# Boey-li/AdaptiGraph

Measured on AMD Instinct MI355X. Metric: rollout graph-steps/s (batch x rollout steps / wall; edge build + GNN forward + state update per graph-step), higher is better.
Workload: dtype f16+fp8corr+bf16x3; 1 GPU; rope 1000+tool particles, batch 256/GPU, 10-step rollout (BASELINE configs[1]); global_batch=256, rollout_steps=10, parallelism=batch-shard x1 + all-gather, rollout_streams=1, weights=seed-0 random init (reference default init), precision=fast, model_status=0, self_edges=1, agg_q16=1

## Files before the change

adaptigraph_amd/csrc/ag_api.hip:

```cpp
#include "../../include/adaptigraph_hip.h"
#include "ag_common.h"

#include <cmath>
#include <cstdarg>
#include <cstdio>
#include <cstdlib>
#include <cstring>
#include <string>
#include <utility>
#include <vector>

namespace {

thread_local std::string g_err;

int fail(int code, const char *fmt, ...)
{
    char buf[512];
    va_list ap;
    va_start(ap, fmt);
    vsnprintf(buf, sizeof buf, fmt, ap);
    va_end(ap);
    g_err = buf;
    return code;
// ... 172 lines not shown
                }
            }
        }
    }
}

}

#define AG_MAX_PARTS 4
struct ag_model {
    ag_model_config cfg;
    float *dev = nullptr;
    size_t dev_floats = 0;
    AgWeights w{};
    int split = 0, fuse_agg = 0, precision = 2, max_blocks = 512, edge_products = 2, edge_ws = 1, node_ws = 1, agg_q16 = 1, node_dedup = 1, self_edges = 1,
        shared_state = 0;
    bool h2_ok = true;
    hipStream_t aux_stream[4] = {nullptr, nullptr, nullptr, nullptr};
    hipEvent_t ev_fork = nullptr, ev_join[4] = {nullptr, nullptr, nullptr, nullptr};
    int cu_split = 0;
    int n_cus = 256;
    int part_cus = 0;
    hipStream_t mfma_stream = nullptr, hbm_stream = nullptr;
    hipEvent_t ev_ready[4] = {nullptr, nullptr, nullptr, nullptr}, ev_enc[4] = {nullptr, nullptr, nullptr, nullptr}, ev_join_mfma = nullptr;
    bool profiling = false;
    std::vector<std::pair<hipEvent_t, hipEvent_t>> ev[AG_K_COUNT];
    size_t ev_used[AG_K_COUNT] = {0, 0, 0, 0, 0, 0};
    unsigned long long *edge_counter = nullptr;
    int *status = nullptr;
};

// ... 222 lines not shown
        r.hs_q16 = (path.q16 && p > 0) ? 1 : 0;
        r.hs_out_q16 = v.hs_q16;
        r.agg_q16 = v.agg_q16;
        if (path.agg_launch) { Timed t(m, AG_K_AGGREGATE, s); ag_launch_aggregate(r, path, last, s); }
        { Timed t(m, AG_K_NODE_UPDATE, s); ag_launch_node_update(m->w, r, path, last, s); }
        std::swap(a.hr, a.hr_out);
        std::swap(a.hs, a.hs_out);
    }
}

struct Option {
    const char *name, *env;
    int ag_model::*field;
    int (*accept)(const ag_model *m, int v);
    const char *takes;
};
int flag(const ag_model *, int v) { return v != 0; }
const Option kOptions[] = {
    {"rollout_streams", "AG_SPLIT", &ag_model::split, [](const ag_model *, int v) { return v >= 0 && v <= AG_MAX_PARTS ? v : -1; }, "0 (by the workload) or 1..4"},
    {"fuse_aggregate", "AG_FUSE_AGG", &ag_model::fuse_agg, [](const ag_model *, int v) { return v == 0 || v == 2 ? v : -1; }, "0 (separate launch) or 2 (reduce inside node_update)"},
    {"precision", "AG_PRECISION", &ag_model::precision, [](const ag_model *, int v) { return v >= 0 && v <= 2 ? v : -1; }, "0 (f32), 1 (bf16x3) or 2 (fast)"},
    {"max_blocks", "AG_MAX_BLOCKS", &ag_model::max_blocks, [](const ag_model *, int v) { return v >= 1 ? v : -1; }, "a positive workgroup count"},
    {"edge_products", "AG_EDGE_PRODUCTS", &ag_model::edge_products, [](const ag_model *, int v) { return v == 2 || v == 3 ? v : -1; }, "2 (fp16 edge stack) or 3 (split-bf16)"},
    {"edge_stationary", "AG_EDGE_WS", &ag_model::edge_ws, flag, "any integer (0 = off)"},
    {"node_stationary", "AG_NODE_WS", &ag_model::node_ws, flag, "any integer (0 = off)"},
    {"agg_q16", "AG_AGG_Q16", &ag_model::agg_q16, flag, "any integer (0 = off)"},
    {"node_dedup", "AG_NODE_DEDUP", &ag_model::node_dedup, [](const ag_model *, int v) { return v < 0 ? 0 : (v > 2 ? 2 : v); }, "any integer (clamped to 0..2)"},
    {"self_edges", "AG_SELF_EDGES", &ag_model::self_edges, flag, "any integer (0 = off)"},
    {"shared_state", "AG_SHARED_STATE", &ag_model::shared_state, flag, "any integer (0 = off)"},
    {"cu_split", "AG_CU_SPLIT", &ag_model::cu_split, [](const ag_model *m, int v) { return v == 0 || (v >= 8 && v <= m->n_cus - 8 && !(v & 7)) ? v : -1; },
     "0 (off) or a multiple of 8 in [8, #CUs - 8]"},
};

const Option *find_option(const char *name)
{
    for (const Option &o : kOptions)
        if (!strcmp(name, o.name)) return &o;
    return nullptr;
}

int load_env_options(ag_model *m)
{
    static const char *const kPrecisionNames[] = {"f32", "bf16x3", "fast"};
    for (const Option &o : kOptions) {
        const char *text = getenv(o.env);
        if (!text) continue;
        char *end = nullptr;
        long long v = strtoll(text, &end, 10);
        bool parsed = *text && !*end && v == (int)v;
        for (int i = 0; i < 3 && !parsed && o.field == &ag_model::precision; ++i)
            if (!strcmp(text, kPrecisionNames[i])) { v = i; parsed = true; }
        const int stored = parsed ? o.accept(m, (int)v) : -1;
        if (stored < 0) return fail(AG_ERR_CONFIG, "%s=%s: %s takes %s", o.env, text, o.name, o.takes);
        m->*o.field = stored;
    }
    return AG_OK;
}

}

// ... 423 lines not shown
                   ag_stream_t stream)
{
    if (!pos || !mask || !tool_mask || !thr_sq || !row_ptr || !edge_recv || !edge_send || !workspace)
        return fail(AG_ERR_ARG, "ag_build_edges: null argument");
    if (B < 1 || N < 1 || topk < 1 || topk > 64) return fail(AG_ERR_ARG, "ag_build_edges: B=%d N=%d topk=%d (1..64)", B, N, topk);
    if (variant != AG_VARIANT_SINGLE && variant != AG_VARIANT_BATCH) return fail(AG_ERR_ARG, "bad variant %d", variant);
    if ((int64_t)B * N >= (1ll << 31) / 64) return fail(AG_ERR_ARG, "B*N too large for int32 edge offsets");
    if (e_cap < ag_edge_capacity(B, N, topk, connect_tools_all, max_tools))
        return fail(AG_ERR_ARG, "ag_build_edges: e_cap %lld < ag_edge_capacity()", (long long)e_cap);
    AgEdgeArgs a{};
    a.pos = pos; a.mask = mask; a.tool = tool_mask; a.thr_sq = thr_sq;
    a.topk = topk; a.connect = connect_tools_all ? 1 : 0; a.variant = variant; a.B = B; a.N = N; a.max_tools = max_tools;
    edge_caps(N, topk, a.connect, max_tools, &a.cap0, &a.cap);
    a.row_ptr = row_ptr; a.edge_recv = edge_recv; a.edge_send = edge_send;
    a.pos_stride = (size_t)N * 3;
    Carver c(workspace, workspace_bytes);
    carve_edges(c, a);
    if (!c.ok()) return fail(AG_ERR_WS, "ag_build_edges: workspace %zu < %zu bytes", workspace_bytes, c.off);
    ag_launch_build_edges(a, static_cast<hipStream_t>(stream));
    AG_HIP(hipGetLastError());
    return AG_OK;
}

size_t ag_forward_workspace_bytes(int B, int N, int64_t e_cap) { return ag_forward_workspace_bytes_for(nullptr, B, N, e_cap); }

size_t ag_forward_workspace_bytes_for(const ag_model *m, int B, int N, int64_t e_cap)
{
    AgFwdArgs a{};
    Carver c(nullptr, 0);
    carve_forward(c, a, B, N, e_cap, resolve_path(m, B, N, 0).q16);
// ... 289 lines not shown
        AG_HIP(hipStreamWaitEvent(sE, m->ev_fork, 0));
        AG_HIP(hipStreamWaitEvent(sR, m->ev_fork, 0));
    }
    int rc = AG_OK;
    struct Run { AgStepArgs st{}; hipStream_t s; } run[AG_MAX_PARTS];
    for (int k = 0; k < parts && rc == AG_OK; ++k) {
        Part &q = part[k];
        hipStream_t s = partitioned ? sR : (k == 0 ? s0 : m->aux_stream[k]);
        run[k].s = s;
        const size_t b0 = (size_t)q.b0;
        const size_t state_bytes = (size_t)q.B * H * plane * sizeof(float);
        if (hipMemcpyAsync(q.state, state0 + b0 * H * plane, state_bytes, hipMemcpyDeviceToDevice, s) != hipSuccess) { rc = AG_ERR_HIP; break; }
        AgEdgeArgs &e = q.e;
        AgFwdArgs &f = q.f;
        e.mask = mask + b0 * N; e.tool = tool_mask + b0 * N; e.thr_sq = thr_sq + b0; e.topk = p->topk;
        e.variant = AG_VARIANT_BATCH; e.max_tools = p->max_tools;
        e.pos = q.state + (size_t)(H - 1) * plane;
        e.pos_stride = (size_t)H * plane;
        f.state = q.state; f.attrs = attrs + b0 * N * 2; f.action = delta + b0 * plane;
        f.p_instance = p_instance + b0 * n_p * p->n_instance; f.phys = phys ? phys + b0 * Pd : nullptr;
        f.row_ptr = e.row_ptr; f.edge_recv = e.edge_recv; f.edge_send = e.edge_send;
        f.pred_pos = q.pp; f.pred_motion = q.pm;
        f.B = q.B; f.N = N; f.n_p = n_p; f.n_inst = p->n_instance; f.phys_dim = Pd;
        f.pstep = m->cfg.pstep; f.clamp = m->cfg.motion_clamp;
        if (m->self_edges) {
            e.self_attrs = f.attrs; e.self_class_row0 = f.self_class_row0;
            f.self_info = e.self_info; f.self_rows = AG_SELF_ROWS;
        }
        AgStepArgs &st = run[k].st;
        st.state = q.state; st.delta = delta + b0 * plane; st.pred_pos = q.pp;
        st.obj_mask = obj_mask ? obj_mask + b0 * n_p : nullptr; st.repeat = repeat + b0;
// ... 9 lines not shown
        for (int k = 0; k < parts && rc == AG_OK && p->n_steps > 0; ++k) {
            AgFwdArgs &f = part[k].f;
            { Timed tm(m, AG_K_EDGES, sR); ag_launch_build_edges(part[k].e, sR); }
            setup_args(m, f, part[k].path, AG_MLP_WG_PER_CU * (m->n_cus - m->cu_split));
            f.ws_blocks = m->cu_split;
            run_node_encode(m, f, sR);
            run_node_encode_fallback(m, f, sR);
            rc = encode(k);
        }
        for (int ai = 1; ai <= p->n_steps && rc == AG_OK; ++ai)
            for (int k = 0; k < parts && rc == AG_OK; ++k) {
                AgFwdArgs &f = part[k].f;
                if (hipStreamWaitEvent(sR, m->ev_enc[k], 0) != hipSuccess) { rc = AG_ERR_HIP; break; }
                run_propagate(m, f, part[k].path, sR);
                run[k].st.step = ai;
                { Timed tm(m, AG_K_ROLLOUT_STEP, sR); ag_launch_rollout_step(run[k].st, sR); }
                if (ai < p->n_steps) {
                    { Timed tm(m, AG_K_EDGES, sR); ag_launch_build_edges(part[k].e, sR); }
                    if (!f.dedup) run_node_encode(m, f, sR);
                    run_node_encode_fallback(m, f, sR);
                    rc = encode(k);
                }
            }
    } else
    for (int ai = 1; ai <= p->n_steps && rc == AG_OK; ++ai)
        for (int k = 0; k < parts && rc == AG_OK; ++k) {
            hipStream_t s = run[k].s;
            AgFwdArgs &f = part[k].f;
            AgEdgeArgs &e = part[k].e;
            const AgPath &path = part[k].path;
            if (ai == 1) {
                setup_args(m, f, path, part_blocks);
                if (path.edge == AG_EDGE_H3_WS) {
                    e.tab_state = f.state; e.tab_attrs = f.attrs; e.tab_pinst = f.p_instance; e.tab_out = f.edge_node_tab;
                    e.tab_n_inst = f.n_inst; e.tab_n_p = f.n_p; e.tab_status = f.status;
                }
                if (f.dedup) { e.map_node_row = f.node_row; e.map_ovf = f.ovf; e.map_send_c = f.send_c; }
            }
            if (ai == 1 || !f.dedup) run_node_encode(m, f, s);
            int riders;
            { Timed tm(m, AG_K_EDGES, s); riders = ag_launch_build_edges(e, s); }
            f.tab_done = (riders & AG_RIDER_TAB) != 0;
            f.remap_done = (riders & AG_RIDER_MAP) != 0;
            run_node_encode_fallback(m, f, s);
            run_edge_encode(m, f, path, s);
            if (ai == 1 && k == 0 && parts > 1) {
                if (hipEventRecord(m->ev_fork, s0) != hipSuccess) { rc = AG_ERR_HIP; break; }
                for (int kk = 1; kk < parts; ++kk)
                    if (hipStreamWaitEvent(m->aux_stream[kk], m->ev_fork, 0) != hipSuccess) rc = AG_ERR_HIP;
                if (rc != AG_OK) break;
            }
            run_propagate(m, f, path, s);
            run[k].st.step = ai;
            { Timed tm(m, AG_K_ROLLOUT_STEP, s); ag_launch_rollout_step(run[k].st, s); }
        }
    for (int k = 0; k < parts && rc == AG_OK && state_final; ++k) {
        const size_t b0 = (size_t)part[k].b0;
        if (hipMemcpyAsync(state_final + b0 * H * plane, part[k].state, (size_t)part[k].B * H * plane * sizeof(float),
                           hipMemcpyDeviceToDevice, run[k].s) != hipSuccess)
            rc = AG_ERR_HIP;
    }
    if (partitioned) {
        if (hipEventRecord(m->ev_join_mfma, sE) != hipSuccess || hipStreamWaitEvent(s0, m->ev_join_mfma, 0) != hipSuccess ||
            hipEventRecord(m->ev_join[1], sR) != hipSuccess || hipStreamWaitEvent(s0, m->ev_join[1], 0) != hipSuccess)
            rc = AG_ERR_HIP;
    } else
    for (int k = 1; k < parts; ++k)
        if (hipEventRecord(m->ev_join[k], m->aux_stream[k]) != hipSuccess || hipStreamWaitEvent(s0, m->ev_join[k], 0) != hipSuccess)
            rc = AG_ERR_HIP;
// ... 7 lines not shown
```

adaptigraph_amd/csrc/ag_common.h:

```cpp
#pragma once
#include <hip/hip_runtime.h>
#include <stdint.h>

#define AG_F 150
#define AG_FP 160
#define AG_NT 5
#define AG_WSTRIDE 160
#define AG_CHUNK_FLOATS 5120
#define AG_CHUNK_F4 1280
#define AG_ROWS_PER_WAVE 32
#ifndef AG_MLP_THREADS
#define AG_MLP_THREADS 256
#endif
#define AG_MLP_WAVES (AG_MLP_THREADS / 64)
#define AG_ROWS_PER_BLOCK (32 * AG_MLP_WAVES)
#define AG_MLP_WG_PER_CU (512 / AG_MLP_THREADS)
#define AG_PACK_BLOCK (32 * AG_FP)
#define AG_NHIS 4
#define AG_ATTR 2
#define AG_EDGE_IN 17
#define AG_NODE_IN_MAX 8

enum { AG_PREC_F32 = 0, AG_PREC_B3 = 1 };
enum { AG_OK = 0, AG_ERR_ARG = -1, AG_ERR_HIP = -2, AG_ERR_WS = -3, AG_ERR_CONFIG = -4 };
// ... 264 lines not shown
    void *grid_raw;
    int32_t *cell_start;
    float4 *sorted;
    const float *tab_state, *tab_attrs, *tab_pinst;
    float *tab_out;
    int tab_n_inst, tab_n_p;
    int *tab_status;
    const int32_t *map_node_row;
    const int *map_ovf;
    int32_t *map_send_c;
    const float *self_attrs;
    int32_t *self_info;
    int32_t *self_pos;
    int self_class_row0;
    const int32_t *active;
};
enum { AG_RIDER_TAB = 1, AG_RIDER_MAP = 2 };
int ag_launch_build_edges(const AgEdgeArgs &a, hipStream_t s);

__device__ __forceinline__ void ag_edge_node_tab_row(const float *state, const float *attrs, const float *p_instance, int n_inst, int n_p,
                                                     int B, int N, float *tab, int *status, int g, long long class_row0 = -1)
{
    if (class_row0 >= 0 && g < AG_SELF_CLASSES) {
        float4 *dst = reinterpret_cast<float4 *>(tab + (size_t)(class_row0 + g) * 16);
        dst[0] = make_float4(g == 0 ? 1.0f : 0.0f, g == 0 ? 0.0f : 1.0f, 0.0f, 0.0f);
        dst[1] = dst[2] = dst[3] = make_float4(0.0f, 0.0f, 0.0f, 0.0f);
    }
    if (g >= B * N) return;
    const int b = g / N, i = g - b * N;
    float p[AG_NHIS][3];
#pragma unroll
    for (int hh = 0; hh < AG_NHIS; ++hh)
#pragma unroll
// ... 19 lines not shown

struct AgStepArgs {
    float *state;
    const float *delta;
    const float *pred_pos;
    const int32_t *cmap;
    uint8_t *dirty;
    int32_t *sample_dirty;
    const uint8_t *obj_mask;
    const int32_t *repeat;
    float *out_seq;
    int B, N, n_p, H, step, height_mode;
    float raise;
};
void ag_launch_rollout_step(const AgStepArgs &a, hipStream_t s);
void ag_launch_zero_words(int32_t *p, int n, hipStream_t s);

struct AgSharedArgs {
    int B1, N, n_p, n_inst, phys_dim, H;
    const float *state0, *delta, *attrs, *p_instance, *phys, *thr_sq;
    const uint8_t *mask, *tool, *obj_mask;
    const int32_t *repeat;
    float *s_state, *s_delta, *s_attrs, *s_pinst, *s_phys, *s_thr;
    uint8_t *s_mask, *s_tool, *s_obj_mask;
    int32_t *s_repeat;
    uint8_t *dirty;
    uint8_t *sel_a, *sel_b;
    int32_t *sample_dirty;
    int32_t *active;
    int max_tools;
// ... 47 lines not shown
```

adaptigraph_amd/csrc/ag_edges.hip:

```cpp
#include "ag_common.h"

namespace {

constexpr int kRowsPerBlock = 16;
constexpr int kCand = 384;

__device__ __forceinline__ void wave_lds_fence()
{
    asm volatile("s_waitcnt lgkmcnt(0)" ::: "memory");
    __builtin_amdgcn_wave_barrier();
}

__device__ int prune_topk(float *cd, int *cj, int cnt, int k, int lane)
{
    unsigned keepbits = 0;
    for (int base = 0, ch = 0; base < cnt; base += 64, ++ch) {
        const int idx = base + lane;
        const bool have = idx < cnt;
        const float d = have ? cd[idx] : 0.f;
        const int jj = have ? cj[idx] : 0;
        int rank = 0;
        for (int t = 0; t < cnt; ++t) {
            const float dt = cd[t];
            const int jt = cj[t];
// ... 106 lines not shown
    *total = wsum[0] + wsum[1] + wsum[2] + wsum[3];
    __syncthreads();
    return base + x - v;
}

constexpr int kCellMax = 8192;

struct GridParams { float x0, y0, z0, inv; int nx, ny, nz, total; };

__device__ __forceinline__ int cell_coord(float x, float x0, float inv, int n)
{
    const int c = (int)((x - x0) * inv);
    return c < 0 ? 0 : (c >= n ? n - 1 : c);
}

__global__ __launch_bounds__(256) void bin_kernel(AgEdgeArgs a)
{
    __shared__ int cnt[kCellMax];
    __shared__ float red[6][4];
    __shared__ GridParams G;
    if ((int)blockIdx.x >= a.B) {
        const int gt = ((int)blockIdx.x - a.B) * 256 + (int)threadIdx.x;
        if (a.active && gt < a.B * a.N && !a.active[gt / a.N]) return;
        ag_edge_node_tab_row(a.tab_state, a.tab_attrs, a.tab_pinst, a.tab_n_inst, a.tab_n_p, a.B, a.N, a.tab_out, a.tab_status, gt,
                             a.self_attrs ? (long long)a.self_class_row0 : -1);
        return;
    }
    if (a.active && !a.active[blockIdx.x]) return;
    const int b = blockIdx.x, N = a.N, tid = threadIdx.x, lane = tid & 63, wave = tid >> 6;
    const float *pos = a.pos + (size_t)b * a.pos_stride;
// ... 32 lines not shown
        lo[1] = fminf(lo[1], y); hi[1] = fmaxf(hi[1], y);
        lo[2] = fminf(lo[2], z); hi[2] = fmaxf(hi[2], z);
    });
    for (int c = 0; c < 3; ++c) {
        for (int o = 32; o > 0; o >>= 1) { lo[c] = fminf(lo[c], __shfl_xor(lo[c], o)); hi[c] = fmaxf(hi[c], __shfl_xor(hi[c], o)); }
        if (lane == 0) { red[c][wave] = lo[c]; red[3 + c][wave] = hi[c]; }
    }
    __syncthreads();
    if (tid == 0) {
        float mn[3], mx[3];
        for (int c = 0; c < 3; ++c) {
            mn[c] = fminf(fminf(red[c][0], red[c][1]), fminf(red[c][2], red[c][3]));
            mx[c] = fmaxf(fmaxf(red[3 + c][0], red[3 + c][1]), fmaxf(red[3 + c][2], red[3 + c][3]));
            if (!(mx[c] >= mn[c])) { mn[c] = 0.f; mx[c] = 0.f; }
        }
        float cs = sqrtf(a.thr_sq[b]) * 1.002f;
        if (!(cs > 1e-20f)) cs = 1e-20f;
        int nx = 1, ny = 1, nz = 1;
        bool ok = true;
        for (int c = 0; c < 3; ++c) ok = ok && isfinite(mn[c]) && isfinite(mx[c]) && isfinite(mx[c] - mn[c]);
        for (int it = 0; ok; ++it) {
            const float fx = (mx[0] - mn[0]) / cs, fy = (mx[1] - mn[1]) / cs, fz = (mx[2] - mn[2]) / cs;
            if (fx < 8000.f && fy < 8000.f && fz < 8000.f) {
                nx = (int)fx + 1; ny = (int)fy + 1; nz = (int)fz + 1;
                if ((long long)nx * ny * nz <= kCellMax) break;
            }
            cs *= 2.0f;
            if (it > 300 || !isfinite(cs)) ok = false;
        }
        if (!ok) { nx = ny = nz = 1; cs = 1.0f; for (int c = 0; c < 3; ++c) if (!isfinite(mn[c])) mn[c] = 0.f; }
        G.x0 = mn[0]; G.y0 = mn[1]; G.z0 = mn[2]; G.inv = 1.0f / cs; G.nx = nx; G.ny = ny; G.nz = nz; G.total = 0;
    }
    __syncthreads();
    if (a.connect && tid == 0) a.flag[b] = 0;
    const GridParams g = G;
    const int ncell = g.nx * g.ny * g.nz;
    for (int c = tid; c < ncell; c += 256) cnt[c] = 0;
    __syncthreads();
    for_valid([&](int, float x, float y, float z, bool) {
        const int cid = (cell_coord(z, g.z0, g.inv, g.nz) * g.ny + cell_coord(y, g.y0, g.inv, g.ny)) * g.nx + cell_coord(x, g.x0, g.inv, g.nx);
        atomicAdd(&cnt[cid], 1);
    });
    __syncthreads();
    int local = 0;
    for (int c = tid * 32; c < tid * 32 + 32 && c < ncell; ++c) local += cnt[c];
    int total;
// ... 170 lines not shown
    bool hit = false;
#pragma unroll
    for (int s = 0; s < K; ++s)
        if (s < cnt) {
            int rank = 0;
#pragma unroll
            for (int t = 0; t < K; ++t) rank += (t < cnt && bj[t] < bj[s]) ? 1 : 0;
            a.sel0[row * a.cap0 + rank] = bj[s];
            hit = hit || (ti && !tl[bj[s]]);
        }
    a.deg[row] = cnt;
    if (a.connect && a.variant == 1 && hit) atomicOr(&a.flag[b], 1);
}

template <int K>
__global__ __launch_bounds__(256, 4) void select_lanes_packed_kernel(AgEdgeArgs a, int jb)
{
    const int b = blockIdx.y, N = a.N;
    if (a.active && !a.active[b]) return;
    const int t = blockIdx.x * 256 + threadIdx.x;
    const uint8_t *mk = a.mask + (size_t)b * N, *tl = a.tool + (size_t)b * N;
    if (t < N && !mk[t]) a.deg[(size_t)b * N + t] = 0;
    const GridParams g = reinterpret_cast<const GridParams *>(a.grid_raw)[b];
    const int32_t *cstart = a.cell_start + (size_t)b * (kCellMax + 1);
    const float4 *sorted = a.sorted + (size_t)b * N;
    const float thr = a.thr_sq[b];
    const bool active = t < g.total;
    const float4 me = active ? sorted[t] : make_float4(0.f, 0.f, 0.f, 0.f);
    const int wi = __float_as_int(me.w);
    const int i = wi & 0x3fffffff;
    const bool ti = (wi & 0x40000000) != 0;
    const float xi = me.x, yi = me.y, zi = me.z;
    const unsigned jmask = (1u << jb) - 1u;
    const float qmax = (float)(1u << (32 - jb));
    const float qscale = qmax / thr;
    const unsigned qtop = (1u << (32 - jb)) - 1u;
    unsigned kl[K + 1];
#pragma unroll
    for (int s = 0; s <= K; ++s) kl[s] = 0xffffffffu;
    int tot = 0;
    if (active) {
        const int ix = cell_coord(xi, g.x0, g.inv, g.nx), iy = cell_coord(yi, g.y0, g.inv, g.ny), iz = cell_coord(zi, g.z0, g.inv, g.nz);
        const int x_lo = ix > 0 ? ix - 1 : 0, x_hi = ix + 1 < g.nx ? ix + 1 : g.nx - 1;
        for (int r = 0; r < 9; ++r) {
            const int z2 = iz + r / 3 - 1, y2 = iy + r % 3 - 1;
            if (z2 < 0 || z2 >= g.nz || y2 < 0 || y2 >= g.ny) continue;
            const int base = (z2 * g.ny + y2) * g.nx;
            const int p1 = cstart[base + x_hi + 1];
            for (int p = cstart[base + x_lo]; p < p1; p += 4) {
                float4 sq[4];
#pragma unroll
                for (int u = 0; u < 4; ++u) sq[u] = sorted[p + u < p1 ? p + u : p1 - 1];
#pragma unroll
                for (int u = 0; u < 4; ++u) {
                    if (p + u >= p1) break;
                    const float4 sj = sq[u];
                    const int w = __float_as_int(sj.w);
                    const float dx = xi - sj.x, dy = yi - sj.y, dz = zi - sj.z;
                    float d = (dx * dx + dy * dy) + dz * dz;
                    if (ti && (w & 0x40000000)) d = 1e10f;
                    if ((d - thr) < 0.0f) {
                        const unsigned qd = min((unsigned)(d * qscale), qtop);
                        unsigned key = (qd << jb) | (unsigned)(w & 0x3fffffff);
#pragma unroll
                        for (int s = 0; s <= K; ++s) {
                            const unsigned lo = min(kl[s], key);
                            key = max(kl[s], key);
                            kl[s] = lo;
                        }
                        ++tot;
                    }
                }
            }
        }
    }
    int cnt = tot < K ? tot : K;
    const bool ambiguous = tot > K && ((kl[K - 1] ^ kl[K]) & ~jmask) == 0u;
    if (__ballot(ambiguous)) {
        float bd[K];
        int bj[K];
        const int c2 = lanes_exact<K>(ambiguous, xi, yi, zi, ti, g, cstart, sorted, thr, bd, bj);
        if (ambiguous) {
            cnt = c2;
#pragma unroll
            for (int s = 0; s < K; ++s) kl[s] = (unsigned)bj[s];
        }
    }
    unsigned js[K];
#pragma unroll
    for (int s = 0; s < K; ++s) js[s] = s < cnt ? (kl[s] & (ambiguous ? 0x7fffffffu : jmask)) : 0x7fffffffu;
#pragma unroll
    for (int round = 0; round < K; ++round)
#pragma unroll
        for (int s = round & 1; s + 1 < K; s += 2) {
            const unsigned lo = min(js[s], js[s + 1]), hi = max(js[s], js[s + 1]);
            js[s] = lo;
            js[s + 1] = hi;
        }
    if (!active) return;
    const size_t row = (size_t)b * N + i;
    bool hit = false;
#pragma unroll
    for (int s = 0; s < K; ++s)
        if (s < cnt) {
            a.sel0[row * a.cap0 + s] = (int)js[s];
            hit = hit || (ti && !tl[js[s]]);
        }
    a.deg[row] = cnt;
    if (a.connect && a.variant == 1 && hit) atomicOr(&a.flag[b], 1);
}

constexpr int kKeepFast = 8;
constexpr int kToolListMax = 8192;
// ... 256 lines not shown
            e[u] = s_ptr[lr] + slot - (slot > s_self[lr] ? 1 : 0);
            sg[u] = (row / a.N) * a.N + v[u];
            a.edge_recv[e[u]] = row;
            a.edge_send[e[u]] = sg[u];
        }
        if (map) {
#pragma unroll
            for (int u = 0; u < 4; ++u) rw[u] = ident ? sg[u] : a.map_node_row[sg[u]];
#pragma unroll
            for (int u = 0; u < 4; ++u)
                if (e[u] >= 0) a.map_send_c[e[u]] = rw[u];
        }
    }
}

}

int ag_launch_build_edges(const AgEdgeArgs &a, hipStream_t s)
{
    const int rows = a.B * a.N;
    int riders = 0;
    const bool cells = a.N >= 256;
    if (a.connect && !cells) ag_launch_zero_words(a.flag, a.B, s);
    if (cells) {
        const int nb_tab = a.tab_out ? (rows + 255) / 256 : 0;
        hipLaunchKernelGGL(bin_kernel, dim3(a.B + nb_tab), dim3(256), 0, s, a);
        if (nb_tab) riders |= AG_RIDER_TAB;
        const dim3 lgrid((a.N + 255) / 256, a.B);
        int jb = 1;
        while ((1 << jb) < a.N) ++jb;
        const bool pk = jb <= 16;
        if (a.cap0 == 5 && a.topk == 5) {
            if (pk) hipLaunchKernelGGL(select_lanes_packed_kernel<5>, lgrid, dim3(256), 0, s, a, jb);
            else hipLaunchKernelGGL(select_lanes_kernel<5>, lgrid, dim3(256), 0, s, a);
// ... 30 lines not shown
```

adaptigraph_amd/csrc/ag_rollout.hip:

```cpp
#include "ag_common.h"

namespace {

constexpr int kStepChunk = 2048;

template <bool SHARED>
__global__ __launch_bounds__(256) void rollout_step_kernel(AgStepArgs a)
{
    __shared__ float red[8];
    const int b = blockIdx.x, tid = threadIdx.x, lane = tid & 63, wave = tid >> 6;
    const float *pred = a.pred_pos + (SHARED ? (size_t)0 : (size_t)b * a.n_p * 3);
    const int32_t *cm = SHARED ? a.cmap + (size_t)b * a.N : nullptr;
    auto at = [&](int i, int c) { return SHARED ? pred[(size_t)cm[i] * 3 + c] : pred[i * 3 + c]; };

    float y;
    if (a.height_mode == 0) {
        float m = INFINITY;
        for (int i = tid; i < a.n_p; i += 256) m = fminf(m, at(i, 1));
#pragma unroll
        for (int o = 32; o > 0; o >>= 1) m = fminf(m, __shfl_xor(m, o));
        if (lane == 0) red[wave] = m;
        __syncthreads();
        y = fminf(fminf(red[0], red[1]), fminf(red[2], red[3]));
    } else {
        const uint8_t *mk = a.obj_mask + (size_t)b * a.n_p;
        float s = 0.f, c = 0.f;
        for (int i = tid; i < a.n_p; i += 256) {
            const float w = mk[i] ? 1.f : 0.f;
            s += at(i, 1) * w;
            c += w;
        }
#pragma unroll
        for (int o = 32; o > 0; o >>= 1) { s += __shfl_xor(s, o); c += __shfl_xor(c, o); }
        if (lane == 0) { red[wave] = s; red[4 + wave] = c; }
        __syncthreads();
        y = ((red[0] + red[1]) + (red[2] + red[3])) / ((red[4] + red[5]) + (red[6] + red[7]));
    }
    y += a.raise;

    const int plane = a.N * 3;
    const int k0 = blockIdx.y * kStepChunk, k1 = min(k0 + kStepChunk, plane);
    if (a.repeat[b] == a.step && !(SHARED && b == 0)) {
        float *o = a.out_seq + (size_t)(SHARED ? b - 1 : b) * a.n_p * 3;
        for (int k = k0 + tid; k < min(k1, a.n_p * 3); k += 256) o[k] = SHARED ? at(k / 3, k % 3) : pred[k];
    }
    float *st = a.state + (size_t)b * a.H * a.N * 3;
    const float *dl = a.delta + (size_t)b * a.N * 3;
    auto mark = [&](int n, int c, float v) {
        if constexpr (SHARED)
            if (b > 0 && cm[n] != n && __float_as_uint(v) != __float_as_uint(pred[(size_t)n * 3 + c])) { a.dirty[(size_t)b * a.N + n] = 1; a.sample_dirty[b] = 1; }
    };
    if (a.H == AG_NHIS) {
        constexpr int kPer = kStepChunk / 256;
// ... 53 lines not shown
```

Before: 159,700 graph-steps/s.

## Fuse rollout state update and per-sample edge build into one workgroup kernel

Adds a fused edge-build path in which one 1024-thread workgroup per sample applies the previous rollout step's state shift, builds the spatial grid in LDS, selects top-k neighbours, and scans degrees. A small finish kernel then writes global CSR offsets. This replaces the separate rollout-step launch and the multi-kernel bin/select/scan edge pipeline for small N, cutting launches and global round trips. The cost is heavy LDS use and one block per sample (B=256 blocks), which may underuse the GPU. It also adds more code paths for the state-update ordering to stay correct.

```diff
diff --git a/adaptigraph_amd/csrc/ag_api.hip b/adaptigraph_amd/csrc/ag_api.hip
--- a/adaptigraph_amd/csrc/ag_api.hip
+++ b/adaptigraph_amd/csrc/ag_api.hip
@@ -210,7 +210,7 @@
     size_t dev_floats = 0;
     AgWeights w{};
     int split = 0, fuse_agg = 0, precision = 2, max_blocks = 512, edge_products = 2, edge_ws = 1, node_ws = 1, agg_q16 = 1, node_dedup = 1, self_edges = 1,
-        shared_state = 0;
+        shared_state = 0, edges_fused = 1;
     bool h2_ok = true;
     hipStream_t aux_stream[4] = {nullptr, nullptr, nullptr, nullptr};
     hipEvent_t ev_fork = nullptr, ev_join[4] = {nullptr, nullptr, nullptr, nullptr};
@@ -463,6 +463,7 @@
     int ag_model::*field;
     int (*accept)(const ag_model *m, int v);
     const char *takes;
+    bool from_env = true;
 };
 int flag(const ag_model *, int v) { return v != 0; }
 const Option kOptions[] = {
@@ -477,6 +478,7 @@
     {"node_dedup", "AG_NODE_DEDUP", &ag_model::node_dedup, [](const ag_model *, int v) { return v < 0 ? 0 : (v > 2 ? 2 : v); }, "any integer (clamped to 0..2)"},
     {"self_edges", "AG_SELF_EDGES", &ag_model::self_edges, flag, "any integer (0 = off)"},
     {"shared_state", "AG_SHARED_STATE", &ag_model::shared_state, flag, "any integer (0 = off)"},
+    {"edges_fused", "AG_EDGES_FUSED", &ag_model::edges_fused, flag, "any integer (0 = off)", false},
     {"cu_split", "AG_CU_SPLIT", &ag_model::cu_split, [](const ag_model *m, int v) { return v == 0 || (v >= 8 && v <= m->n_cus - 8 && !(v & 7)) ? v : -1; },
      "0 (off) or a multiple of 8 in [8, #CUs - 8]"},
 };
@@ -492,7 +494,7 @@
 {
     static const char *const kPrecisionNames[] = {"f32", "bf16x3", "fast"};
     for (const Option &o : kOptions) {
-        const char *text = getenv(o.env);
+        const char *text = o.from_env ? getenv(o.env) : nullptr;
         if (!text) continue;
         char *end = nullptr;
         long long v = strtoll(text, &end, 10);
@@ -946,6 +948,7 @@
     edge_caps(N, topk, a.connect, max_tools, &a.cap0, &a.cap);
     a.row_ptr = row_ptr; a.edge_recv = edge_recv; a.edge_send = edge_send;
     a.pos_stride = (size_t)N * 3;
+    a.fused = 1;
     Carver c(workspace, workspace_bytes);
     carve_edges(c, a);
     if (!c.ok()) return fail(AG_ERR_WS, "ag_build_edges: workspace %zu < %zu bytes", workspace_bytes, c.off);
@@ -1265,7 +1268,7 @@
         AgEdgeArgs &e = q.e;
         AgFwdArgs &f = q.f;
         e.mask = mask + b0 * N; e.tool = tool_mask + b0 * N; e.thr_sq = thr_sq + b0; e.topk = p->topk;
-        e.variant = AG_VARIANT_BATCH; e.max_tools = p->max_tools;
+        e.variant = AG_VARIANT_BATCH; e.max_tools = p->max_tools; e.fused = m->edges_fused;
         e.pos = q.state + (size_t)(H - 1) * plane;
         e.pos_stride = (size_t)H * plane;
         f.state = q.state; f.attrs = attrs + b0 * N * 2; f.action = delta + b0 * plane;
@@ -1305,9 +1308,10 @@
                 if (hipStreamWaitEvent(sR, m->ev_enc[k], 0) != hipSuccess) { rc = AG_ERR_HIP; break; }
                 run_propagate(m, f, part[k].path, sR);
                 run[k].st.step = ai;
-                { Timed tm(m, AG_K_ROLLOUT_STEP, sR); ag_launch_rollout_step(run[k].st, sR); }
+                const bool carried = ai < p->n_steps && ag_edges_fused(part[k].e);
+                if (!carried) { Timed tm(m, AG_K_ROLLOUT_STEP, sR); ag_launch_rollout_step(run[k].st, sR); }
                 if (ai < p->n_steps) {
-                    { Timed tm(m, AG_K_EDGES, sR); ag_launch_build_edges(part[k].e, sR); }
+                    { Timed tm(m, AG_K_EDGES, sR); ag_launch_build_edges(part[k].e, sR, carried ? &run[k].st : nullptr); }
                     if (!f.dedup) run_node_encode(m, f, sR);
                     run_node_encode_fallback(m, f, sR);
                     rc = encode(k);
@@ -1330,7 +1334,7 @@
             }
             if (ai == 1 || !f.dedup) run_node_encode(m, f, s);
             int riders;
-            { Timed tm(m, AG_K_EDGES, s); riders = ag_launch_build_edges(e, s); }
+            { Timed tm(m, AG_K_EDGES, s); riders = ag_launch_build_edges(e, s, ai > 1 && ag_edges_fused(e) ? &run[k].st : nullptr); }
             f.tab_done = (riders & AG_RIDER_TAB) != 0;
             f.remap_done = (riders & AG_RIDER_MAP) != 0;
             run_node_encode_fallback(m, f, s);
@@ -1343,7 +1347,7 @@
             }
             run_propagate(m, f, path, s);
             run[k].st.step = ai;
-            { Timed tm(m, AG_K_ROLLOUT_STEP, s); ag_launch_rollout_step(run[k].st, s); }
+            if (ai == p->n_steps || !ag_edges_fused(e)) { Timed tm(m, AG_K_ROLLOUT_STEP, s); ag_launch_rollout_step(run[k].st, s); }
         }
     for (int k = 0; k < parts && rc == AG_OK && state_final; ++k) {
         const size_t b0 = (size_t)part[k].b0;
diff --git a/adaptigraph_amd/csrc/ag_common.h b/adaptigraph_amd/csrc/ag_common.h
--- a/adaptigraph_amd/csrc/ag_common.h
+++ b/adaptigraph_amd/csrc/ag_common.h
@@ -302,9 +302,20 @@
     int32_t *self_pos;
     int self_class_row0;
     const int32_t *active;
+    int fused;
 };
 enum { AG_RIDER_TAB = 1, AG_RIDER_MAP = 2 };
-int ag_launch_build_edges(const AgEdgeArgs &a, hipStream_t s);
+#define AG_FUSED_MAX_N 1024
+#define AG_FUSED_CELLS 2048
+#define AG_FUSED_LDS_BUDGET 65536
+inline size_t ag_edges_fused_lds_bytes(int N, int cap)
+{
+    const size_t Np = ((size_t)N + 63) & ~(size_t)63;
+    return Np * (16 + 12 + 4 + 4 + 1) + 4 * (2 * (size_t)AG_FUSED_CELLS + 1) + 4 * (size_t)cap + 16;
+}
+struct AgStepArgs;
+bool ag_edges_fused(const AgEdgeArgs &a);
+int ag_launch_build_edges(const AgEdgeArgs &a, hipStream_t s, const AgStepArgs *prev = nullptr);
 
 __device__ __forceinline__ void ag_edge_node_tab_row(const float *state, const float *attrs, const float *p_instance, int n_inst, int n_p,
                                                      int B, int N, float *tab, int *status, int g, long long class_row0 = -1)
@@ -354,6 +365,39 @@
     float raise;
 };
 void ag_launch_rollout_step(const AgStepArgs &a, hipStream_t s);
+template <class At>
+__device__ __forceinline__ float ag_step_tool_height(const AgStepArgs &a, int b, At at, float *red)
+{
+    const int tid = threadIdx.x, lane = tid & 63, wave = tid >> 6;
+    float y;
+    if (a.height_mode == 0) {
+        if (tid < 256) {
+            float m = INFINITY;
+            for (int i = tid; i < a.n_p; i += 256) m = fminf(m, at(i, 1));
+#pragma unroll
+            for (int o = 32; o > 0; o >>= 1) m = fminf(m, __shfl_xor(m, o));
+            if (lane == 0) red[wave] = m;
+        }
+        __syncthreads();
+        y = fminf(fminf(red[0], red[1]), fminf(red[2], red[3]));
+    } else {
+        if (tid < 256) {
+            const uint8_t *mk = a.obj_mask + (size_t)b * a.n_p;
+            float s = 0.f, c = 0.f;
+            for (int i = tid; i < a.n_p; i += 256) {
+                const float w = mk[i] ? 1.f : 0.f;
+                s += at(i, 1) * w;
+                c += w;
+            }
+#pragma unroll
+            for (int o = 32; o > 0; o >>= 1) { s += __shfl_xor(s, o); c += __shfl_xor(c, o); }
+            if (lane == 0) { red[wave] = s; red[4 + wave] = c; }
+        }
+        __syncthreads();
+        y = ((red[0] + red[1]) + (red[2] + red[3])) / ((red[4] + red[5]) + (red[6] + red[7]));
+    }
+    return y + a.raise;
+}
 void ag_launch_zero_words(int32_t *p, int n, hipStream_t s);
 
 struct AgSharedArgs {
diff --git a/adaptigraph_amd/csrc/ag_edges.hip b/adaptigraph_amd/csrc/ag_edges.hip
--- a/adaptigraph_amd/csrc/ag_edges.hip
+++ b/adaptigraph_amd/csrc/ag_edges.hip
@@ -144,6 +144,28 @@
     return c < 0 ? 0 : (c >= n ? n - 1 : c);
 }
 
+__device__ GridParams make_grid(float (&mn)[3], float (&mx)[3], float thr_sq, int cell_max)
+{
+    GridParams G;
+    float cs = sqrtf(thr_sq) * 1.002f;
+    if (!(cs > 1e-20f)) cs = 1e-20f;
+    int nx = 1, ny = 1, nz = 1;
+    bool ok = true;
+    for (int c = 0; c < 3; ++c) ok = ok && isfinite(mn[c]) && isfinite(mx[c]) && isfinite(mx[c] - mn[c]);
+    for (int it = 0; ok; ++it) {
+        const float fx = (mx[0] - mn[0]) / cs, fy = (mx[1] - mn[1]) / cs, fz = (mx[2] - mn[2]) / cs;
+        if (fx < 8000.f && fy < 8000.f && fz < 8000.f) {
+            nx = (int)fx + 1; ny = (int)fy + 1; nz = (int)fz + 1;
+            if ((long long)nx * ny * nz <= cell_max) break;
+        }
+        cs *= 2.0f;
+        if (it > 300 || !isfinite(cs)) ok = false;
+    }
+    if (!ok) { nx = ny = nz = 1; cs = 1.0f; for (int c = 0; c < 3; ++c) if (!isfinite(mn[c])) mn[c] = 0.f; }
+    G.x0 = mn[0]; G.y0 = mn[1]; G.z0 = mn[2]; G.inv = 1.0f / cs; G.nx = nx; G.ny = ny; G.nz = nz; G.total = 0;
+    return G;
+}
+
 __global__ __launch_bounds__(256) void bin_kernel(AgEdgeArgs a)
 {
     __shared__ int cnt[kCellMax];
@@ -206,22 +228,7 @@
             mx[c] = fmaxf(fmaxf(red[3 + c][0], red[3 + c][1]), fmaxf(red[3 + c][2], red[3 + c][3]));
             if (!(mx[c] >= mn[c])) { mn[c] = 0.f; mx[c] = 0.f; }
         }
-        float cs = sqrtf(a.thr_sq[b]) * 1.002f;
-        if (!(cs > 1e-20f)) cs = 1e-20f;
-        int nx = 1, ny = 1, nz = 1;
-        bool ok = true;
-        for (int c = 0; c < 3; ++c) ok = ok && isfinite(mn[c]) && isfinite(mx[c]) && isfinite(mx[c] - mn[c]);
-        for (int it = 0; ok; ++it) {
-            const float fx = (mx[0] - mn[0]) / cs, fy = (mx[1] - mn[1]) / cs, fz = (mx[2] - mn[2]) / cs;
-            if (fx < 8000.f && fy < 8000.f && fz < 8000.f) {
-                nx = (int)fx + 1; ny = (int)fy + 1; nz = (int)fz + 1;
-                if ((long long)nx * ny * nz <= kCellMax) break;
-            }
-            cs *= 2.0f;
-            if (it > 300 || !isfinite(cs)) ok = false;
-        }
-        if (!ok) { nx = ny = nz = 1; cs = 1.0f; for (int c = 0; c < 3; ++c) if (!isfinite(mn[c])) mn[c] = 0.f; }
-        G.x0 = mn[0]; G.y0 = mn[1]; G.z0 = mn[2]; G.inv = 1.0f / cs; G.nx = nx; G.ny = ny; G.nz = nz; G.total = 0;
+        G = make_grid(mn, mx, a.thr_sq[b], kCellMax);
     }
     __syncthreads();
     if (a.connect && tid == 0) a.flag[b] = 0;
@@ -422,6 +429,78 @@
 }
 
 template <int K>
+__device__ __forceinline__ int select_packed_row(bool active, float xi, float yi, float zi, bool ti, const GridParams &g, const int32_t *cstart,
+                                                 const float4 *sorted, float thr, int jb, unsigned (&js)[K])
+{
+    const unsigned jmask = (1u << jb) - 1u;
+    const float qmax = (float)(1u << (32 - jb));
+    const float qscale = qmax / thr;
+    const unsigned qtop = (1u << (32 - jb)) - 1u;
+    unsigned kl[K + 1];
+#pragma unroll
+    for (int s = 0; s <= K; ++s) kl[s] = 0xffffffffu;
+    int tot = 0;
+    if (active) {
+        const int ix = cell_coord(xi, g.x0, g.inv, g.nx), iy = cell_coord(yi, g.y0, g.inv, g.ny), iz = cell_coord(zi, g.z0, g.inv, g.nz);
+        const int x_lo = ix > 0 ? ix - 1 : 0, x_hi = ix + 1 < g.nx ? ix + 1 : g.nx - 1;
+        for (int r = 0; r < 9; ++r) {
+            const int z2 = iz + r / 3 - 1, y2 = iy + r % 3 - 1;
+            if (z2 < 0 || z2 >= g.nz || y2 < 0 || y2 >= g.ny) continue;
+            const int base = (z2 * g.ny + y2) * g.nx;
+            const int p1 = cstart[base + x_hi + 1];
+            for (int p = cstart[base + x_lo]; p < p1; p += 4) {
+                float4 sq[4];
+#pragma unroll
+                for (int u = 0; u < 4; ++u) sq[u] = sorted[p + u < p1 ? p + u : p1 - 1];
+#pragma unroll
+                for (int u = 0; u < 4; ++u) {
+                    if (p + u >= p1) break;
+                    const float4 sj = sq[u];
+                    const int w = __float_as_int(sj.w);
+                    const float dx = xi - sj.x, dy = yi - sj.y, dz = zi - sj.z;
+                    float d = (dx * dx + dy * dy) + dz * dz;
+                    if (ti && (w & 0x40000000)) d = 1e10f;
+                    if ((d - thr) < 0.0f) {
+                        const unsigned qd = min((unsigned)(d * qscale), qtop);
+                        unsigned key = (qd << jb) | (unsigned)(w & 0x3fffffff);
+#pragma unroll
+                        for (int s = 0; s <= K; ++s) {
+                            const unsigned lo = min(kl[s], key);
+                            key = max(kl[s], key);
+                            kl[s] = lo;
+                        }
+                        ++tot;
+                    }
+                }
+            }
+        }
+    }
+    int cnt = tot < K ? tot : K;
+    const bool ambiguous = tot > K && ((kl[K - 1] ^ kl[K]) & ~jmask) == 0u;
+    if (__ballot(ambiguous)) {
+        float bd[K];
+        int bj[K];
+        const int c2 = lanes_exact<K>(ambiguous, xi, yi, zi, ti, g, cstart, sorted, thr, bd, bj);
+        if (ambiguous) {
+            cnt = c2;
+#pragma unroll
+            for (int s = 0; s < K; ++s) kl[s] = (unsigned)bj[s];
+        }
+    }
+#pragma unroll
+    for (int s = 0; s < K; ++s) js[s] = s < cnt ? (kl[s] & (ambiguous ? 0x7fffffffu : jmask)) : 0x7fffffffu;
+#pragma unroll
+    for (int round = 0; round < K; ++round)
+#pragma unroll
+        for (int s = round & 1; s + 1 < K; s += 2) {
+            const unsigned lo = min(js[s], js[s + 1]), hi = max(js[s], js[s + 1]);
+            js[s] = lo;
+            js[s + 1] = hi;
+        }
+    return cnt;
+}
+
+template <int K>
 __global__ __launch_bounds__(256, 4) void select_lanes_packed_kernel(AgEdgeArgs a, int jb)
 {
     const int b = blockIdx.y, N = a.N;
@@ -439,72 +518,8 @@
     const int i = wi & 0x3fffffff;
     const bool ti = (wi & 0x40000000) != 0;
     const float xi = me.x, yi = me.y, zi = me.z;
-    const unsigned jmask = (1u << jb) - 1u;
-    const float qmax = (float)(1u << (32 - jb));
-    const float qscale = qmax / thr;
-    const unsigned qtop = (1u << (32 - jb)) - 1u;
-    unsigned kl[K + 1];
-#pragma unroll
-    for (int s = 0; s <= K; ++s) kl[s] = 0xffffffffu;
-    int tot = 0;
-    if (active) {
-        const int ix = cell_coord(xi, g.x0, g.inv, g.nx), iy = cell_coord(yi, g.y0, g.inv, g.ny), iz = cell_coord(zi, g.z0, g.inv, g.nz);
-        const int x_lo = ix > 0 ? ix - 1 : 0, x_hi = ix + 1 < g.nx ? ix + 1 : g.nx - 1;
-        for (int r = 0; r < 9; ++r) {
-            const int z2 = iz + r / 3 - 1, y2 = iy + r % 3 - 1;
-            if (z2 < 0 || z2 >= g.nz || y2 < 0 || y2 >= g.ny) continue;
-            const int base = (z2 * g.ny + y2) * g.nx;
-            const int p1 = cstart[base + x_hi + 1];
-            for (int p = cstart[base + x_lo]; p < p1; p += 4) {
-                float4 sq[4];
-#pragma unroll
-                for (int u = 0; u < 4; ++u) sq[u] = sorted[p + u < p1 ? p + u : p1 - 1];
-#pragma unroll
-                for (int u = 0; u < 4; ++u) {
-                    if (p + u >= p1) break;
-                    const float4 sj = sq[u];
-                    const int w = __float_as_int(sj.w);
-                    const float dx = xi - sj.x, dy = yi - sj.y, dz = zi - sj.z;
-                    float d = (dx * dx + dy * dy) + dz * dz;
-                    if (ti && (w & 0x40000000)) d = 1e10f;
-                    if ((d - thr) < 0.0f) {
-                        const unsigned qd = min((unsigned)(d * qscale), qtop);
-                        unsigned key = (qd << jb) | (unsigned)(w & 0x3fffffff);
-#pragma unroll
-                        for (int s = 0; s <= K; ++s) {
-                            const unsigned lo = min(kl[s], key);
-                            key = max(kl[s], key);
-                            kl[s] = lo;
-                        }
-                        ++tot;
-                    }
-                }
-            }
-        }
-    }
-    int cnt = tot < K ? tot : K;
-    const bool ambiguous = tot > K && ((kl[K - 1] ^ kl[K]) & ~jmask) == 0u;
-    if (__ballot(ambiguous)) {
-        float bd[K];
-        int bj[K];
-        const int c2 = lanes_exact<K>(ambiguous, xi, yi, zi, ti, g, cstart, sorted, thr, bd, bj);
-        if (ambiguous) {
-            cnt = c2;
-#pragma unroll
-            for (int s = 0; s < K; ++s) kl[s] = (unsigned)bj[s];
-        }
-    }
     unsigned js[K];
-#pragma unroll
-    for (int s = 0; s < K; ++s) js[s] = s < cnt ? (kl[s] & (ambiguous ? 0x7fffffffu : jmask)) : 0x7fffffffu;
-#pragma unroll
-    for (int round = 0; round < K; ++round)
-#pragma unroll
-        for (int s = round & 1; s + 1 < K; s += 2) {
-            const unsigned lo = min(js[s], js[s + 1]), hi = max(js[s], js[s + 1]);
-            js[s] = lo;
-            js[s + 1] = hi;
-        }
+    const int cnt = select_packed_row<K>(active, xi, yi, zi, ti, g, cstart, sorted, thr, jb, js);
     if (!active) return;
     const size_t row = (size_t)b * N + i;
     bool hit = false;
@@ -791,10 +806,296 @@
     }
 }
 
-}
-
-int ag_launch_build_edges(const AgEdgeArgs &a, hipStream_t s)
-{
+__device__ __forceinline__ int block_exclusive_scan_waves(int v, int *wsum, int *total)
+{
+    const int lane = threadIdx.x & 63, wave = threadIdx.x >> 6, nw = blockDim.x >> 6;
+    int x = v;
+#pragma unroll
+    for (int o = 1; o < 64; o <<= 1) {
+        const int y = __shfl_up(x, o);
+        if (lane >= o) x += y;
+    }
+    if (lane == 63) wsum[wave] = x;
+    __syncthreads();
+    int base = 0, all = 0;
+    for (int w = 0; w < nw; ++w) { const int c = wsum[w]; all += c; base += w < wave ? c : 0; }
+    *total = all;
+    __syncthreads();
+    return base + x - v;
+}
+
+constexpr int kFusedPer = 3;
+
+template <int K>
+__global__ __launch_bounds__(1024) void build_sample_kernel(AgEdgeArgs a, AgStepArgs st, int with_step, int jb)
+{
+    extern __shared__ __attribute__((aligned(16))) unsigned char smem[];
+    __shared__ float red[6][16];
+    __shared__ int wsum[16];
+    __shared__ GridParams G;
+    __shared__ int s_flag;
+    const int b = blockIdx.x, N = a.N, tid = threadIdx.x, nthr = blockDim.x, lane = tid & 63, wave = tid >> 6, nw = nthr >> 6;
+    const int Np = (N + 63) & ~63, plane = N * 3;
+    float4 *sorted = reinterpret_cast<float4 *>(smem);
+    float *spos = reinterpret_cast<float *>(sorted + Np);
+    int *deg_l = reinterpret_cast<int *>(spos + 3 * Np);
+    int *ptr_l = deg_l + Np;
+    int *cstart = ptr_l + Np;
+    int *cursor = cstart + AG_FUSED_CELLS + 1;
+    int *tools = cursor + AG_FUSED_CELLS;
+    unsigned char *sflag = reinterpret_cast<unsigned char *>(tools + a.cap);
+    const uint8_t *mk = a.mask + (size_t)b * N, *tl = a.tool + (size_t)b * N;
+
+    if (with_step) {
+        const float *pred = st.pred_pos + (size_t)b * st.n_p * 3;
+        auto at = [&](int i, int c) { return pred[i * 3 + c]; };
+        const float y = ag_step_tool_height(st, b, at, &red[0][0]);
+        if (st.repeat[b] == st.step) {
+            float *o = st.out_seq + (size_t)b * st.n_p * 3;
+            for (int k = tid; k < st.n_p * 3; k += nthr) o[k] = pred[k];
+        }
+        float *sp = st.state + (size_t)b * AG_NHIS * plane;
+        const float *dl = st.delta + (size_t)b * plane;
+        float v[kFusedPer][AG_NHIS], nv[kFusedPer];
+#pragma unroll
+        for (int i = 0; i < kFusedPer; ++i) {
+            const int k = tid + nthr * i;
+            if (k < plane) {
+#pragma unroll
+                for (int h = 1; h < AG_NHIS; ++h) v[i][h] = sp[(size_t)h * plane + k];
+                const int n = k / 3, c = k - n * 3;
+                nv[i] = n < st.n_p ? pred[k] : (c == 1 ? y : v[i][AG_NHIS - 1] + dl[k]);
+            }
+        }
+#pragma unroll
+        for (int i = 0; i < kFusedPer; ++i) {
+            const int k = tid + nthr * i;
+            if (k < plane) {
+#pragma unroll
+                for (int h = 0; h + 1 < AG_NHIS; ++h) sp[(size_t)h * plane + k] = v[i][h + 1];
+                sp[(size_t)(AG_NHIS - 1) * plane + k] = nv[i];
+                spos[k] = nv[i];
+            }
+        }
+    } else {
+        const float *pos = a.pos + (size_t)b * a.pos_stride;
+        for (int k = tid; k < plane; k += nthr) spos[k] = pos[k];
+    }
+    for (int j = tid; j < Np; j += nthr) {
+        sflag[j] = j < N ? (unsigned char)((mk[j] ? 1 : 0) | (tl[j] ? 2 : 0)) : 0;
+        deg_l[j] = 0;
+    }
+    if (tid == 0) s_flag = 0;
+    __syncthreads();
+
+    if (a.tab_out && tid < N)
+        ag_edge_node_tab_row(a.tab_state, a.tab_attrs, a.tab_pinst, a.tab_n_inst, a.tab_n_p, a.B, N, a.tab_out, a.tab_status, b * N + tid,
+                             a.self_attrs ? (long long)a.self_class_row0 : -1);
+
+    const bool valid = tid < N && (sflag[tid < N ? tid : 0] & 1);
+    const bool tool_me = valid && (sflag[tid] & 2);
+    const float px = valid ? spos[tid * 3] : 0.f, py = valid ? spos[tid * 3 + 1] : 0.f, pz = valid ? spos[tid * 3 + 2] : 0.f;
+    {
+        float lo[3] = {valid ? px : INFINITY, valid ? py : INFINITY, valid ? pz : INFINITY};
+        float hi[3] = {valid ? px : -INFINITY, valid ? py : -INFINITY, valid ? pz : -INFINITY};
+        for (int c = 0; c < 3; ++c) { lo[c] = fminf(INFINITY, lo[c]); hi[c] = fmaxf(-INFINITY, hi[c]); }
+        for (int c = 0; c < 3; ++c) {
+            for (int o = 32; o > 0; o >>= 1) { lo[c] = fminf(lo[c], __shfl_xor(lo[c], o)); hi[c] = fmaxf(hi[c], __shfl_xor(hi[c], o)); }
+            if (lane == 0) { red[c][wave] = lo[c]; red[3 + c][wave] = hi[c]; }
+        }
+    }
+    __syncthreads();
+    if (tid == 0) {
+        float mn[3], mx[3];
+        for (int c = 0; c < 3; ++c) {
+            mn[c] = INFINITY; mx[c] = -INFINITY;
+            for (int w = 0; w < nw; ++w) { mn[c] = fminf(mn[c], red[c][w]); mx[c] = fmaxf(mx[c], red[3 + c][w]); }
+            if (!(mx[c] >= mn[c])) { mn[c] = 0.f; mx[c] = 0.f; }
+        }
+        G = make_grid(mn, mx, a.thr_sq[b], AG_FUSED_CELLS);
+    }
+    __syncthreads();
+    GridParams g = G;
+    const int ncell = g.nx * g.ny * g.nz;
+    for (int c = tid; c < ncell; c += nthr) cursor[c] = 0;
+    __syncthreads();
+    const int cid = (cell_coord(pz, g.z0, g.inv, g.nz) * g.ny + cell_coord(py, g.y0, g.inv, g.ny)) * g.nx + cell_coord(px, g.x0, g.inv, g.nx);
+    if (valid) atomicAdd(&cursor[cid], 1);
+    __syncthreads();
+    {
+        const int per = (ncell + nthr - 1) / nthr;
+        int local = 0;
+        for (int c = tid * per; c < tid * per + per && c < ncell; ++c) local += cursor[c];
+        int total;
+        int run = block_exclusive_scan_waves(local, wsum, &total);
+        for (int c = tid * per; c < tid * per + per && c < ncell; ++c) {
+            const int v = cursor[c];
+            cursor[c] = run;
+            cstart[c] = run;
+            run += v;
+        }
+        if (tid == 0) cstart[ncell] = total;
+        g.total = total;
+    }
+    __syncthreads();
+    if (valid) {
+        const int p = atomicAdd(&cursor[cid], 1);
+        sorted[p] = make_float4(px, py, pz, __int_as_float(tid | (tool_me ? 0x40000000 : 0)));
+    }
+    __syncthreads();
+
+    const float thr = a.thr_sq[b];
+    const bool active = tid < g.total;
+    const float4 me = active ? sorted[tid] : make_float4(0.f, 0.f, 0.f, 0.f);
+    const int wi = __float_as_int(me.w);
+    const int i = wi & 0x3fffffff;
+    const bool ti = (wi & 0x40000000) != 0;
+    unsigned js[K];
+    const int cnt = select_packed_row<K>(active, me.x, me.y, me.z, ti, g, cstart, sorted, thr, jb, js);
+
+    int nb = 0;
+    const bool keep_sel = !ti;
+    if (a.connect) {
+        bool hit = false;
+#pragma unroll
+        for (int s = 0; s < K; ++s)
+            if (s < cnt) hit = hit || (ti && !(sflag[js[s]] & 2));
+        if (active && hit) atomicOr(&s_flag, 1);
+        const bool tj = tid < N && (sflag[tid < N ? tid : 0] & 2);
+        const unsigned long long bal = __ballot(tj);
+        if (lane == 0) wsum[wave] = __popcll(bal);
+        __syncthreads();
+        int base = 0, nt = 0;
+        for (int w = 0; w < nw; ++w) { const int c = wsum[w]; nt += c; base += w < wave ? c : 0; }
+        const int slot = base + __popcll(bal & ((1ull << lane) - 1ull));
+        if (tj && slot < a.cap) tools[slot] = tid;
+        __syncthreads();
+        nb = (active && s_flag != 0) ? (nt < a.cap ? nt : a.cap) : 0;
+    }
+    const int caps = a.connect ? a.cap : a.cap0;
+    auto walk = [&](auto &&emit) {
+        int ib = 0;
+#pragma unroll
+        for (int s = 0; s < K; ++s)
+            if (s < cnt && (!a.connect || (keep_sel && !(sflag[js[s]] & 2)))) {
+                while (ib < nb && tools[ib] < (int)js[s]) emit(tools[ib++]);
+                emit((int)js[s]);
+            }
+        while (ib < nb) emit(tools[ib++]);
+    };
+
+    int self_at = -1;
+    if (active) {
+        const size_t row = (size_t)b * N + i;
+        int out = 0, sp = -1;
+        walk([&](int j) { if (out < caps && j == i) sp = out; ++out; });
+        const int deg = out < caps ? out : caps;
+        if (a.self_attrs) {
+            const int cls = ag_self_class(a.self_attrs[row * 2], a.self_attrs[row * 2 + 1]);
+            if (cls >= 0 && sp >= 0 && sp <= 0xffff) self_at = sp;
+            a.self_info[row] = self_at >= 0 ? ((cls << 16) | self_at) : -1;
+        }
+        deg_l[i] = deg - (self_at >= 0 ? 1 : 0);
+    }
+    if (a.self_attrs && tid < N && !(sflag[tid] & 1)) a.self_info[(size_t)b * N + tid] = -1;
+    __syncthreads();
+    {
+        int total;
+        const int ex = block_exclusive_scan_waves(tid < N ? deg_l[tid] : 0, wsum, &total);
+        if (tid < N) { ptr_l[tid] = ex; a.deg[(size_t)b * N + tid] = ex; }
+        if (tid == 0) a.flag[b] = total;
+    }
+    __syncthreads();
+
+    if (active) {
+        int32_t *dst = (a.connect ? a.sel : a.sel0) + (size_t)b * N * caps + ptr_l[i];
+        int out = 0;
+        walk([&](int j) {
+            if (out < caps && out != self_at) dst[out - ((self_at >= 0 && out > self_at) ? 1 : 0)] = (i << 16) | j;
+            ++out;
+        });
+    }
+}
+
+constexpr int kFinishChunk = 2048;
+
+__global__ __launch_bounds__(256) void finish_edges_kernel(AgEdgeArgs a, const int32_t *stage, int caps, int ny)
+{
+    const int g = blockIdx.x, y = blockIdx.y, N = a.N, tid = threadIdx.x;
+    const bool map = a.map_send_c != nullptr;
+    const bool ident = map && *a.map_ovf != 0;
+    int part = 0;
+    for (int i = tid; i < g; i += 256) part += a.flag[i];
+    const int total = a.flag[g];
+    int base;
+    block_exclusive_scan(part, &base);
+    const int rper = (N + ny - 1) / ny, r1 = (y + 1) * rper < N ? (y + 1) * rper : N;
+    for (int i = y * rper + tid; i < r1; i += 256) a.row_ptr[(size_t)g * N + i] = base + a.deg[(size_t)g * N + i];
+    if (g == a.B - 1 && y == 0) {
+        if (tid == 0) a.row_ptr[(size_t)a.B * N] = base + total;
+        if (a.self_attrs && tid < AG_SELF_ROWS) {
+            a.edge_recv[base + total + tid] = a.self_class_row0 + tid / AG_SELF_REPL;
+            a.edge_send[base + total + tid] = a.self_class_row0 + tid / AG_SELF_REPL;
+        }
+    }
+    const int32_t *src = stage + (size_t)g * N * caps;
+    const int e1 = (y + 1) * kFinishChunk < total ? (y + 1) * kFinishChunk : total, node0 = g * N;
+    for (int i0 = y * kFinishChunk + tid; i0 < e1; i0 += 4 * 256) {
+        int w[4], sg[4], rw[4];
+#pragma unroll
+        for (int u = 0; u < 4; ++u) w[u] = i0 + 256 * u < e1 ? src[i0 + 256 * u] : 0;
+#pragma unroll
+        for (int u = 0; u < 4; ++u) {
+            sg[u] = node0 + (w[u] & 0xffff);
+            if (i0 + 256 * u < e1) {
+                a.edge_recv[base + i0 + 256 * u] = node0 + (w[u] >> 16);
+                a.edge_send[base + i0 + 256 * u] = sg[u];
+            }
+        }
+        if (map) {
+#pragma unroll
+            for (int u = 0; u < 4; ++u) rw[u] = ident ? sg[u] : a.map_node_row[sg[u]];
+#pragma unroll
+            for (int u = 0; u < 4; ++u)
+                if (i0 + 256 * u < e1) a.map_send_c[base + i0 + 256 * u] = rw[u];
+        }
+    }
+}
+
+template <int K>
+void launch_fused(const AgEdgeArgs &a, const AgStepArgs *prev, hipStream_t s)
+{
+    int jb = 1;
+    while ((1 << jb) < a.N) ++jb;
+    const int threads = a.N <= 256 ? 256 : (a.N <= 512 ? 512 : 1024);
+    const AgStepArgs st = prev ? *prev : AgStepArgs{};
+    hipLaunchKernelGGL(build_sample_kernel<K>, dim3(a.B), dim3(threads), ag_edges_fused_lds_bytes(a.N, a.cap), s, a, st, prev ? 1 : 0, jb);
+    const int caps = a.connect ? a.cap : a.cap0;
+    const int ny = (int)(((long long)a.N * caps + kFinishChunk - 1) / kFinishChunk);
+    hipLaunchKernelGGL(finish_edges_kernel, dim3(a.B, ny), dim3(256), 0, s, a, a.connect ? a.sel : a.sel0, caps, ny);
+}
+
+}
+
+bool ag_edges_fused(const AgEdgeArgs &a)
+{
+    return a.fused && a.variant == 1 && !a.active && a.N <= AG_FUSED_MAX_N && a.cap0 == a.topk &&
+           (a.topk == 5 || a.topk == 10 || a.topk == 20) && ag_edges_fused_lds_bytes(a.N, a.cap) <= AG_FUSED_LDS_BUDGET;
+}
+
+int ag_launch_build_edges(const AgEdgeArgs &a, hipStream_t s, const AgStepArgs *prev)
+{
+    const bool step_in = prev && !prev->cmap && prev->H == AG_NHIS && prev->B == a.B && prev->N == a.N &&
+                         a.pos == prev->state + (size_t)(AG_NHIS - 1) * a.N * 3 && a.pos_stride == (size_t)AG_NHIS * a.N * 3;
+    if (ag_edges_fused(a)) {
+        if (prev && !step_in) ag_launch_rollout_step(*prev, s);
+        const AgStepArgs *in = step_in ? prev : nullptr;
+        if (a.topk == 5) launch_fused<5>(a, in, s);
+        else if (a.topk == 10) launch_fused<10>(a, in, s);
+        else launch_fused<20>(a, in, s);
+        return (a.tab_out ? AG_RIDER_TAB : 0) | (a.map_send_c ? AG_RIDER_MAP : 0);
+    }
+    if (prev) ag_launch_rollout_step(*prev, s);
     const int rows = a.B * a.N;
     int riders = 0;
     const bool cells = a.N >= 256;
diff --git a/adaptigraph_amd/csrc/ag_rollout.hip b/adaptigraph_amd/csrc/ag_rollout.hip
--- a/adaptigraph_amd/csrc/ag_rollout.hip
+++ b/adaptigraph_amd/csrc/ag_rollout.hip
@@ -8,35 +8,12 @@
 __global__ __launch_bounds__(256) void rollout_step_kernel(AgStepArgs a)
 {
     __shared__ float red[8];
-    const int b = blockIdx.x, tid = threadIdx.x, lane = tid & 63, wave = tid >> 6;
+    const int b = blockIdx.x, tid = threadIdx.x;
     const float *pred = a.pred_pos + (SHARED ? (size_t)0 : (size_t)b * a.n_p * 3);
     const int32_t *cm = SHARED ? a.cmap + (size_t)b * a.N : nullptr;
     auto at = [&](int i, int c) { return SHARED ? pred[(size_t)cm[i] * 3 + c] : pred[i * 3 + c]; };
 
-    float y;
-    if (a.height_mode == 0) {
-        float m = INFINITY;
-        for (int i = tid; i < a.n_p; i += 256) m = fminf(m, at(i, 1));
-#pragma unroll
-        for (int o = 32; o > 0; o >>= 1) m = fminf(m, __shfl_xor(m, o));
-        if (lane == 0) red[wave] = m;
-        __syncthreads();
-        y = fminf(fminf(red[0], red[1]), fminf(red[2], red[3]));
-    } else {
-        const uint8_t *mk = a.obj_mask + (size_t)b * a.n_p;
-        float s = 0.f, c = 0.f;
-        for (int i = tid; i < a.n_p; i += 256) {
-            const float w = mk[i] ? 1.f : 0.f;
-            s += at(i, 1) * w;
-            c += w;
-        }
-#pragma unroll
-        for (int o = 32; o > 0; o >>= 1) { s += __shfl_xor(s, o); c += __shfl_xor(c, o); }
-        if (lane == 0) { red[wave] = s; red[4 + wave] = c; }
-        __syncthreads();
-        y = ((red[0] + red[1]) + (red[2] + red[3])) / ((red[4] + red[5]) + (red[6] + red[7]));
-    }
-    y += a.raise;
+    const float y = ag_step_tool_height(a, b, at, red);
 
     const int plane = a.N * 3;
     const int k0 = blockIdx.y * kStepChunk, k1 = min(k0 + kStepChunk, plane);
```

Result: no change. 160,000 graph-steps/s, median of 4 (+0.2%).
